# DanielaCourel/smoothed_particle_hydrodynamics

Measured on AMD Instinct MI355X. Metric: Mparticle-steps/sec (whole node), dam-break, higher is better.
Workload: dtype f32

## Files before the change

smoothed_particle_hydrodynamics_amd/csrc/cell_build.h:

```cpp
#pragma once

#include "sph_device.h"

#define SCAN_THREADS 256
#ifndef RANK_UNROLL
#define RANK_UNROLL 4
#endif
#ifndef RANK_BIG
#define RANK_BIG 512
#endif
#define RANK_CHUNK 4096
#define RANK_BIG_BLOCKS 64
#define SCAN_ITEMS 16
#define SCAN_TILE (SCAN_THREADS * SCAN_ITEMS)

__device__ __forceinline__ void count_cell_runs(uint32_t c, bool live, int i,
                                                uint32_t* __restrict__ cell_count,
                                                uint32_t* __restrict__ slot, uint32_t trash)
{
   live = live && c != trash;
   const int lane = threadIdx.x & (SPH_WAVE - 1);
   const uint32_t prev = __shfl_up(c, 1);
   const bool head = (lane == 0) || (prev != c);
   const unsigned long long heads = __ballot(head);
   const unsigned long long below = heads & ((lane == 63) ? ~0ull : ((1ull << (lane + 1)) - 1ull));
   const int head_lane = 63 - __clzll(below);
   const unsigned long long above = (head_lane == 63) ? 0ull : (heads >> (head_lane + 1));
   const int run_len = above ? (__ffsll((long long)above)) : (SPH_WAVE - head_lane);
   uint32_t base = 0;
   if (live && head) base = atomicAdd(&cell_count[c], (uint32_t)run_len);
   base = __shfl(base, head_lane);
   if (live) slot[i] = base + (uint32_t)(lane - head_lane);
}

template <bool WRITE_VOX, bool CHECK_DEAD>
__global__ void __launch_bounds__(256)
k_hash_count(const float4* __restrict__ posm, const float4* __restrict__ velp,
             int32_t* __restrict__ meta, CellGrid g, SlabZone zone, uint32_t* __restrict__ key,
             uint32_t* __restrict__ slot, uint32_t* __restrict__ cell_count,
             int32_t* __restrict__ vox)
{
   const int i = blockIdx.x * blockDim.x + threadIdx.x;
   const bool live = i < meta[META_N_IN];
   uint32_t c = 0xffffffffu;
   if (live) {
      const float4 p = posm[i];
      int cx, cy, cz;
      c = cell_of(g, p.x, p.y, p.z, cx, cy, cz);
      const bool carried = zone.drop_ghosts && i < meta[META_N_LIVE];
      const int ob = meta[META_OWN_BEGIN], oe = meta[META_OWN_END];
      const bool was_owned = i >= ob && i < oe;
      if (CHECK_DEAD && __float_as_uint(velp[i].w) == SPH_DEAD_ID) {
         c = (uint32_t)g.ncells;
      } else if (carried && !was_owned) {
         c = (uint32_t)g.ncells;
      } else if (c == (uint32_t)g.ncells) {
         if (!carried) atomicOr(&meta[META_ERRORS], 1);
      } else if (zone.early && carried) {
         const int lo_end = meta[META_BND_LO_END];
         const int hi_begin = max(meta[META_BND_HI_BEGIN], lo_end);
         if (i >= lo_end && i < hi_begin) {
            const int plane = cell_coord(p.z, g.inv, g.nz_global);
            if ((zone.have_left && plane < zone.lo + zone.halo) ||
                (zone.have_right && plane >= zone.hi - zone.halo))
               atomicOr(&meta[META_ERRORS], 8);
// ... 79 lines not shown
      for (int k = 0; k < SCAN_ITEMS / 4; k++) {
         const uint4 q = p[k];
         v[4 * k + 0] = q.x;
         v[4 * k + 1] = q.y;
         v[4 * k + 2] = q.z;
         v[4 * k + 3] = q.w;
      }
   } else {
#pragma unroll
      for (int k = 0; k < SCAN_ITEMS; k++) v[k] = (base + k < ncells) ? count[base + k] : 0u;
   }
#pragma unroll
   for (int k = 0; k < SCAN_ITEMS; k++) s += v[k];
   uint32_t before = 0;
   for (int t = threadIdx.x; t < (int)blockIdx.x; t += SCAN_THREADS) before += part[t];
   uint32_t carry;
   block_exclusive_scan(before, &carry);
   uint32_t total;
   uint32_t run = carry + block_exclusive_scan(s, &total);
   if (base + SCAN_ITEMS <= ncells) {
      uint4* o = reinterpret_cast<uint4*>(cell_start + base);
      uint4* z = reinterpret_cast<uint4*>(count + base);
#pragma unroll
      for (int k = 0; k < SCAN_ITEMS / 4; k++) {
         uint4 q;
         q.x = min(run, limit); run += v[4 * k + 0];
         q.y = min(run, limit); run += v[4 * k + 1];
         q.z = min(run, limit); run += v[4 * k + 2];
         q.w = min(run, limit); run += v[4 * k + 3];
         o[k] = q;
         if ((v[4 * k + 0] | v[4 * k + 1] | v[4 * k + 2] | v[4 * k + 3]) != 0u) z[k] = make_uint4(0, 0, 0, 0);
      }
   } else {
      for (int k = 0; k < SCAN_ITEMS; k++) {
         if (base + k < ncells) {
            cell_start[base + k] = min(run, limit);
            if (v[k] != 0u) count[base + k] = 0;
            run += v[k];
         }
      }
   }
   if (base <= ncells - 1 && ncells - 1 < base + SCAN_ITEMS) {
      cell_start[ncells] = min(run, limit);
      if (run > limit) atomicOr(&meta[META_ERRORS], 4);
   }
}

__global__ void __launch_bounds__(256)
k_scatter(const uint32_t* __restrict__ key, const uint32_t* __restrict__ slot,
          const uint32_t* __restrict__ cell_start, int32_t* __restrict__ meta,
          uint32_t* __restrict__ perm, int cells_per_plane, int ncells, int own_lo, int own_hi,
          int sum_lo, int sum_hi, int bnd_lo, int bnd_hi, int32_t* __restrict__ tile_stats,
          int32_t* __restrict__ clear_a, int32_t* __restrict__ clear_b,
          uint32_t* __restrict__ big_cells, uint32_t limit)
{
   const int i = blockIdx.x * blockDim.x + threadIdx.x;
   if (tile_stats && i < TSTAT_COUNT && i != TSTAT_BLOCKS) tile_stats[i] = 0;
   const int n_in = meta[META_N_IN];
   if (i < n_in) {
      const uint32_t c = key[i];
      if (c != (uint32_t)ncells) {
         const uint32_t first = cell_start[c], sl = slot[i];
         if (first + sl < limit) perm[first + sl] = (uint32_t)i;
         if (sl == 0u && cell_start[c + 1] - first > (uint32_t)RANK_BIG)
            big_cells[1u + atomicAdd(&big_cells[0], 1u)] = c;
      }
   }
   if (i == 0) {
      meta[META_N_LIVE] = (int)cell_start[ncells];
      meta[META_OWN_BEGIN] = (int)cell_start[own_lo * cells_per_plane];
      meta[META_OWN_END] = (int)cell_start[own_hi * cells_per_plane];
      meta[META_SUM_BEGIN] = (int)cell_start[sum_lo * cells_per_plane];
      meta[META_SUM_END] = (int)cell_start[sum_hi * cells_per_plane];
      meta[META_BND_LO_END] = (int)cell_start[bnd_lo * cells_per_plane];
      meta[META_BND_HI_BEGIN] = (int)cell_start[bnd_hi * cells_per_plane];
      if (clear_a) *clear_a = 0;
      if (clear_b) *clear_b = 0;
      if (tile_stats)
         tile_stats[TSTAT_BLOCKS] =
            (meta[META_SUM_END] - meta[META_SUM_BEGIN] + TILE_THREADS - 1) / TILE_THREADS;
   }
}

__global__ void __launch_bounds__(256)
k_rank_order(const uint32_t* __restrict__ perm, const uint32_t* __restrict__ key,
             const uint32_t* __restrict__ cell_start, const int32_t* __restrict__ meta,
             uint32_t* __restrict__ order)
{
   const int p = blockIdx.x * blockDim.x + threadIdx.x;
   if (p >= meta[META_N_IN]) return;
   const uint32_t i = perm[p];
   const uint32_t c = key[i];
   const uint32_t s = cell_start[c], e = cell_start[c + 1];
   if (e - s > (uint32_t)RANK_BIG) return;
   uint32_t rank = 0;
   for (uint32_t q0 = s; q0 < e; q0 += 8) {
      uint32_t other[8];
#pragma unroll
      for (int u = 0; u < 8; u++) other[u] = perm[q0 + u < e ? q0 + u : e - 1];
#pragma unroll
      for (int u = 0; u < 8; u++) rank += (q0 + u < e && other[u] < i) ? 1u : 0u;
   }
   order[s + rank] = i;
}

__device__ __forceinline__ void
rank_gather(int p, int block_p0, uint32_t* __restrict__ lds_id, const uint32_t* __restrict__ perm,
            const uint32_t* __restrict__ key, const uint32_t* __restrict__ cell_start,
            const int32_t* __restrict__ meta, int trash, const float4* __restrict__ posm_in,
            const float4* __restrict__ velp_in, float4* __restrict__ posm_out,
            float4* __restrict__ velp_out, uint32_t* __restrict__ remap = nullptr)
{
   const int n_in = (int)cell_start[trash];
   bool active = p < n_in;
   uint32_t i = 0, c = 0, s = 0, e = 0, id = 0;
   float4 v = make_float4(0.f, 0.f, 0.f, 0.f);
   if (active) {
      i = perm[p];
      c = key[i];
      v = velp_in[i];
      id = __float_as_uint(v.w);
   }
   lds_id[threadIdx.x] = id;
   if (active) {
      if (c == (uint32_t)trash) {
         active = false;
      } else {
         s = cell_start[c];
         e = cell_start[c + 1];
         if (e - s > (uint32_t)RANK_BIG) active = false;
      }
   }
   __syncthreads();
   if (!active) return;
   const uint32_t b0 = (uint32_t)block_p0;
   const uint32_t b1 = min(b0 + blockDim.x, (uint32_t)n_in);
   const uint32_t in_lo = max(s, b0), in_hi = min(e, b1);
   uint32_t rank = 0, same = 0;
   for (uint32_t q0 = in_lo; q0 < in_hi; q0 += 4) {
      uint32_t other[4];
#pragma unroll
      for (int u = 0; u < 4; u++) other[u] = lds_id[(q0 + u < in_hi ? q0 + u : in_hi - 1) - b0];
#pragma unroll
      for (int u = 0; u < 4; u++) {
         rank += (q0 + u < in_hi && other[u] < id) ? 1u : 0u;
         same += (q0 + u < in_hi && other[u] == id) ? 1u : 0u;
      }
   }
#pragma unroll
   for (int side = 0; side < 2; side++) {
      const uint32_t lo = side == 0 ? s : in_hi, hi = side == 0 ? in_lo : e;
      for (uint32_t q0 = lo; q0 < hi; q0 += RANK_UNROLL) {
         uint32_t other[RANK_UNROLL];
#pragma unroll
         for (int u = 0; u < RANK_UNROLL; u++) other[u] = perm[q0 + u < hi ? q0 + u : hi - 1];
#pragma unroll
         for (int u = 0; u < RANK_UNROLL; u++) other[u] = __float_as_uint(velp_in[other[u]].w);
#pragma unroll
         for (int u = 0; u < RANK_UNROLL; u++) {
            rank += (q0 + u < hi && other[u] < id) ? 1u : 0u;
            same += (q0 + u < hi && other[u] == id) ? 1u : 0u;
         }
      }
   }
   if (same > 1u) atomicOr(const_cast<int32_t*>(&meta[META_ERRORS]), 16);
   posm_out[s + rank] = posm_in[i];
   velp_out[s + rank] = v;
   if (remap) remap[i] = s + rank;
}

__global__ void __launch_bounds__(256)
k_rank_gather(const uint32_t* __restrict__ perm, const uint32_t* __restrict__ key,
              const uint32_t* __restrict__ cell_start, const int32_t* __restrict__ meta, int trash,
              const float4* __restrict__ posm_in, const float4* __restrict__ velp_in,
              float4* __restrict__ posm_out, float4* __restrict__ velp_out,
              uint32_t* __restrict__ remap)
{
   __shared__ uint32_t lds_id[256];
   rank_gather(blockIdx.x * blockDim.x + threadIdx.x, blockIdx.x * blockDim.x, lds_id, perm, key,
               cell_start, meta, trash, posm_in, velp_in, posm_out, velp_out, remap);
}

template <bool FULL>
__global__ void __launch_bounds__(256)
k_rank_big(const uint32_t* __restrict__ big_cells, const uint32_t* __restrict__ perm,
           const uint32_t* __restrict__ cell_start, const float4* __restrict__ posm_in,
           const float4* __restrict__ velp_in, float4* __restrict__ posm_out,
           float4* __restrict__ velp_out, uint32_t* __restrict__ order,
           uint32_t* __restrict__ scratch_key, uint32_t* __restrict__ scratch_src,
           uint32_t* __restrict__ remap)
{
   __shared__ uint32_t skey[RANK_CHUNK], ssrc[RANK_CHUNK];
   const int tid = threadIdx.x;
   const uint32_t nbig = big_cells[0];
   for (uint32_t b = blockIdx.x; b < nbig; b += gridDim.x) {
      const uint32_t c = big_cells[1u + b];
      const uint32_t s = cell_start[c], m = cell_start[c + 1] - s;
      const uint32_t nchunks = (m + RANK_CHUNK - 1) / RANK_CHUNK;
      for (uint32_t ch = 0; ch < nchunks; ch++) {
         const uint32_t base = ch * RANK_CHUNK;
         const uint32_t len = min((uint32_t)RANK_CHUNK, m - base);
         uint32_t padded = 256;
         while (padded < len) padded <<= 1;
         for (uint32_t t = tid; t < padded; t += 256) {
            uint32_t key = 0xffffffffu, src = 0u;
            if (t < len) {
               src = perm[s + base + t];
               key = FULL ? __float_as_uint(velp_in[src].w) : src;
            }
            skey[t] = key;
            ssrc[t] = src;
         }
         __syncthreads();
         for (uint32_t k2 = 2; k2 <= padded; k2 <<= 1) {
            for (uint32_t j = k2 >> 1; j > 0; j >>= 1) {
               for (uint32_t t = tid; t < padded; t += 256) {
                  const uint32_t partner = t ^ j;
                  if (partner > t) {
                     const bool up = (t & k2) == 0;
                     const uint32_t a = skey[t], bb = skey[partner];
                     if ((a > bb) == up) {
                        skey[t] = bb;
                        skey[partner] = a;
                        const uint32_t sa = ssrc[t];
                        ssrc[t] = ssrc[partner];
                        ssrc[partner] = sa;
                     }
                  }
               }
               __syncthreads();
            }
         }
         for (uint32_t t = tid; t < len; t += 256) {
            if (nchunks == 1) {
               const uint32_t src = ssrc[t];
               if (FULL) {
                  posm_out[s + t] = posm_in[src];
                  velp_out[s + t] = velp_in[src];
                  if (remap) remap[src] = s + t;
               } else {
                  order[s + t] = src;
               }
            } else {
               scratch_key[s + base + t] = skey[t];
               scratch_src[s + base + t] = ssrc[t];
            }
         }
         __syncthreads();
      }
      if (nchunks > 1) {
         for (uint32_t idx = tid; idx < m; idx += 256) {
            const uint32_t key = scratch_key[s + idx], mine = idx / RANK_CHUNK;
            uint32_t rank = idx % RANK_CHUNK;
            for (uint32_t ch = 0; ch < nchunks; ch++) {
               if (ch == mine) continue;
               const uint32_t* keys = scratch_key + s + ch * RANK_CHUNK;
               uint32_t lo = 0, hi = min((uint32_t)RANK_CHUNK, m - ch * RANK_CHUNK);
               while (lo < hi) {
                  const uint32_t mid = (lo + hi) >> 1;
                  if (keys[mid] < key) lo = mid + 1;
                  else hi = mid;
               }
               rank += lo;
            }
            const uint32_t src = scratch_src[s + idx];
            if (FULL) {
               posm_out[s + rank] = posm_in[src];
               velp_out[s + rank] = velp_in[src];
               if (remap) remap[src] = s + rank;
            } else {
               order[s + rank] = src;
            }
         }
         __syncthreads();
      }
   }
}

__global__ void __launch_bounds__(256)
k_permute_sums(const uint32_t* __restrict__ remap, const uint32_t* __restrict__ key,
               const int32_t* __restrict__ meta, uint32_t trash, const float* __restrict__ rho,
               const float4* __restrict__ acc, const int32_t* __restrict__ ncount,
               float* __restrict__ rho_out, float4* __restrict__ acc_out,
               int32_t* __restrict__ ncount_out)
{
   const int i = blockIdx.x * blockDim.x + threadIdx.x;
   if (i >= meta[META_N_IN] || key[i] == trash) return;
   const uint32_t j = remap[i];
   rho_out[j] = rho[i];
   acc_out[j] = acc[i];
   ncount_out[j] = ncount[i];
}
```

smoothed_particle_hydrodynamics_amd/csrc/context.h:

```cpp
#pragma once

#include <stdlib.h>
#include <string.h>

#include <memory>
#include <new>
#include <utility>

#include "cell_build.h"
#include "common_kernels.h"
#include "full_kernels.h"
#include "full_tiled.h"
#include "ref_kernels.h"
#include "sample_kernels.h"
#include "slab_kernels.h"
#include "slab_rccl.h"

namespace {

std::string g_create_error;

inline int div_up(int a, int b) { return (a + b - 1) / b; }

bool getenv_flag(const char* name)
// ... 65 lines not shown

struct SlabComm {
   ncclComm_t comm = nullptr;
   int rank = 0, nranks = 1;
   Stream stream;
   Event packed;
   Event arrived;
   DevBuf<void> send_left, send_right, recv_left, recv_right;
   int capacity_records = 0;
   int active_records = 0;
   size_t bytes = 0;
   DevBuf<int32_t> trim_word;
   bool primed = false;
   long long steps_run = 0;
   DevBuf<int32_t> fill_word;
   PinnedBuf<int32_t> fill_host;
   Event fill_arrived;
   bool fill_pending = false;
   int growths = 0;

   ~SlabComm()
   {
      const RcclApi* api = comm ? rccl_api(nullptr) : nullptr;
      if (api) (void)api->CommDestroy(comm);
   }
};
#define SLAB_GROW_EVERY 16

struct sph_hip_context {
   sph_hip_params prm;
   int mode = 0;
   int device = 0;
   int capacity = 0;
   int n = 0;
   int n_owned = 0;
   DevBuf<int32_t> meta;
   int plane_lo = 0, plane_hi = 0, halo = 0;
   hipStream_t stream = nullptr;
   Stream own_stream;
   Event ev[EV_RING][7];
   long long ev_steps = 0;
   std::string err;

   CellGrid grid;

   DevBuf<float4> posm[2];
   DevBuf<float4> velp[2];
   int cur = 0;

   DevBuf<uint32_t> key;
   DevBuf<uint32_t> slot;
   DevBuf<uint32_t> perm;
   DevBuf<uint32_t> order;
   DevBuf<uint32_t> cell_count;
   DevBuf<uint32_t> cell_start;
   DevBuf<uint32_t> scan_part;
   DevBuf<uint32_t> big_cells;
   int scan_tiles = 0;

   DevBuf<float> rho;
   DevBuf<float4> velB;
   DevBuf<float> auxc;
   DevBuf<float4> acc;
   DevBuf<int32_t> ncount;
   DevBuf<TileDesc> tile_desc;
   DevBuf<uint32_t> nlist;
   DevBuf<uint32_t> nlist_overflow;
   int fast = 0;
   int uniform_mass = 0;
   int use_tiled = 1;
   int prehashed = 0;
   int no_prehash = 0, no_fused_integrate = 0, no_fused_slab = 0;
   Stream chunk_stream;
   Event ev_chunk_fork, ev_chunk_join;
   int chunked_giveups = -1;
   int slab_fused = 0;
   void* slab_msgs[2] = {nullptr, nullptr};
   int slab_msg_capacity = 0;
   int had_exchange = 0;
   int may_hold_dead = 0;
   int early_exchange = 0;
   std::unique_ptr<SlabComm> comm;
   hipStream_t border_stream = nullptr;
   Event ev_density;
   Event ev_border;
   Event ev_pace[2];
   long long steps_enqueued = 0;
   int timing_level = 2;
   int timing_stride = 1;
   long long timing_seen = 0;
   int slab_step_level = 0;
   PinnedBuf<int> tile_feedback;
   DevBuf<int32_t> tile_stats;
   DevBuf<uint32_t> giveup_density;
   DevBuf<uint32_t> giveup_accel;
   int tile_cap_forced = 0;
   int tile_cap_accel = 0, tile_cap_density = 0;
   int list_cap = 0;
   int list_cap_max = 0;
   size_t list_blocks = 0;
   TileLevels density_levels = {}, accel_levels = {};
   TileCaps caps = {};
   int cand_kept[TILE_CANDS] = {0}, n_cand_kept = 0;

   DevBuf<int32_t> vox;
   DevBuf<uint32_t> nb;
// ... 123 lines not shown
   for (int b = 0; b < nbuf; b++) {
      CREATE_TRY(dev_alloc(ctx->posm[b], cap));
      CREATE_TRY(dev_alloc(ctx->velp[b], cap));
   }
   CREATE_TRY(dev_alloc(ctx->key, cap));
   CREATE_TRY(dev_alloc(ctx->slot, cap));
   CREATE_TRY(dev_alloc(ctx->perm, cap));
   const size_t cells_padded = (size_t)ctx->scan_tiles * SCAN_TILE + 16;
   CREATE_TRY(dev_alloc(ctx->cell_count, cells_padded));
   CREATE_TRY(dev_alloc(ctx->cell_start, cells_padded));
   CREATE_TRY(dev_alloc(ctx->scan_part, (size_t)ctx->scan_tiles + 1));
   CREATE_TRY(dev_alloc(ctx->big_cells, cap / RANK_BIG + 2));
   CREATE_TRY(hipMemsetAsync(ctx->big_cells, 0, sizeof(uint32_t), ctx->stream));
   CREATE_TRY(hipMemsetAsync(ctx->cell_count, 0, cells_padded * sizeof(uint32_t), ctx->stream));
   CREATE_TRY(hipMemsetAsync(ctx->cell_start, 0, cells_padded * sizeof(uint32_t), ctx->stream));
   CREATE_TRY(dev_alloc(ctx->rho, cap));
   CREATE_TRY(dev_alloc(ctx->acc, cap));
   CREATE_TRY(dev_alloc(ctx->ncount, cap));
   CREATE_TRY(hipMemsetAsync(ctx->rho, 0, cap * sizeof(float), ctx->stream));
   CREATE_TRY(hipMemsetAsync(ctx->acc, 0, cap * sizeof(float4), ctx->stream));
   CREATE_TRY(hipMemsetAsync(ctx->ncount, 0, cap * sizeof(int32_t), ctx->stream));
   CREATE_TRY(dev_alloc(ctx->meta, META_COUNT));
   CREATE_TRY(hipMemsetAsync(ctx->meta, 0, META_COUNT * sizeof(int32_t), ctx->stream));
   if (mode == SPH_HIP_MODE_FULL) {
      CREATE_TRY(dev_alloc(ctx->velB, cap));
      CREATE_TRY(dev_alloc(ctx->auxc, cap));
      CREATE_TRY(dev_alloc(ctx->tile_desc, (size_t)div_up(capacity, TILE_THREADS) + 1));
      ctx->list_cap = NLIST_CAP;
      ctx->list_cap_max = NLIST_CAP_MAX;
      if (const char* v = getenv("SPH_HIP_LIST_CAP")) {
         const int c = atoi(v) / 2 * 2;
         if (c > 0) ctx->list_cap = ctx->list_cap_max = c < 2 ? 2 : (c > NLIST_CAP_MAX ? NLIST_CAP_MAX : c);
      }
      ctx->list_blocks = (size_t)div_up(capacity, TILE_THREADS) + 1;
      const size_t nlist_words = ctx->list_blocks * list_rows(ctx->list_cap) * TILE_THREADS;
      CREATE_TRY(dev_alloc(ctx->nlist, nlist_words));
      CREATE_TRY(hipMemsetAsync(ctx->nlist, 0, nlist_words * sizeof(uint32_t), ctx->stream));
      CREATE_TRY(dev_alloc(ctx->nlist_overflow, (size_t)div_up(capacity, TILE_THREADS) + 1));
      if (const char* v = getenv("SPH_HIP_UNTILED")) ctx->use_tiled = (v[0] == '1') ? 0 : 1;
      CREATE_TRY(pinned_alloc(ctx->tile_feedback, TSTAT_COUNT));
      memset(ctx->tile_feedback, 0, TSTAT_COUNT * sizeof(int));
      CREATE_TRY(dev_alloc(ctx->tile_stats, TSTAT_COUNT));
      CREATE_TRY(hipMemsetAsync(ctx->tile_stats, 0, TSTAT_COUNT * sizeof(int32_t), ctx->stream));
      CREATE_TRY(dev_alloc(ctx->giveup_density, (size_t)div_up(capacity, TILE_THREADS) + 1));
      CREATE_TRY(dev_alloc(ctx->giveup_accel, (size_t)div_up(capacity, TILE_THREADS) + 1));
      CREATE_TRY(event_create(ctx->ev_density));
      CREATE_TRY(event_create(ctx->ev_border));
      if (const char* v = getenv("SPH_HIP_TILE_CAP")) {
         const int c = atoi(v);
         if (c > 0) ctx->tile_cap_forced = c < 256 ? 256 : (c > 8000 ? 8000 : c / 32 * 32);
      }
      if (const char* v = getenv("SPH_HIP_TILE_CAP_ACCEL")) ctx->tile_cap_accel = atoi(v) / 32 * 32;
      if (const char* v = getenv("SPH_HIP_TILE_CAP_DENSITY")) ctx->tile_cap_density = atoi(v) / 32 * 32;
   } else {
      CREATE_TRY(dev_alloc(ctx->order, cap));
      CREATE_TRY(dev_alloc(ctx->vox, cap * 3));
      CREATE_TRY(dev_alloc(ctx->nb, cap * (size_t)params->examine_count));
      CREATE_TRY(dev_alloc(ctx->nd, cap * (size_t)params->examine_count));
   }
   CREATE_TRY(dev_alloc(ctx->epart, (size_t)2 * ctx->eblocks + 2));
   CREATE_TRY(hipMemsetAsync(ctx->epart, 0, sizeof(double) * 2, ctx->stream));
   CREATE_TRY(dev_alloc(ctx->stats, 4));
   CREATE_TRY(pinned_alloc(ctx->err_watch, 4));
   for (int i = 0; i < 4; i++) ctx->err_watch[i] = 0;
   CREATE_TRY(event_create(ctx->watch_event));
   CREATE_TRY(dev_alloc(ctx->stage, cap * 12));
   CREATE_TRY(hipStreamSynchronize(ctx->stream));
#undef CREATE_TRY
   *out = ctx.release();
   return SPH_HIP_OK;
}

void destroy_impl(sph_hip_context* ctx)
{
   (void)hipSetDevice(ctx->device);
   if (ctx->stream) (void)hipStreamSynchronize(ctx->stream);
   if (ctx->comm && ctx->comm->stream) (void)hipStreamSynchronize(ctx->comm->stream);
   if (ctx->chunk_stream) (void)hipStreamSynchronize(ctx->chunk_stream);
   if (ctx->copy_stream) (void)hipStreamSynchronize(ctx->copy_stream);
   delete ctx;
}

}
```

smoothed_particle_hydrodynamics_amd/csrc/full_tiled.h:

```cpp
#pragma once

#include "launch_policy.h"
#include "common_kernels.h"
#include "full_kernels.h"
#include "slab_kernels.h"

#if defined(SPH_ABLATE) && !defined(SPH_DIAGNOSTIC_BUILD)
#error "SPH_ABLATE is for diagnostic builds only: add -DSPH_DIAGNOSTIC_BUILD (tools/build_variant.sh does)"
#endif

#ifdef SPH_TRIPCOUNT
#ifndef SPH_DIAGNOSTIC_BUILD
#error "SPH_TRIPCOUNT is for diagnostic builds only: add -DSPH_DIAGNOSTIC_BUILD"
#endif
enum {
   TRIP_D_WAVES = 0, TRIP_D_CHUNKS_W, TRIP_D_TEST8_W, TRIP_D_TEST8_L, TRIP_D_SLOTS_L, TRIP_D_POPS_W,
   TRIP_D_POPS_L, TRIP_D_POPLOOPS_W, TRIP_D_SUMTRIPS_W, TRIP_D_SUMSLOTS_W, TRIP_D_LISTED_L, TRIP_D_LANES_L,
   TRIP_A_WAVES = 16, TRIP_A_PTRIPS_W, TRIP_A_CNT_L, TRIP_A_VTRIPS_W, TRIP_A_NV_L, TRIP_A_LANES_L,
   TRIP_COUNT = 32
};
__device__ unsigned long long g_trip[TRIP_COUNT];
struct TripCounters {
   unsigned int v[16];
   __device__ TripCounters() { for (int i = 0; i < 16; i++) v[i] = 0; }
// ... 181 lines not shown
         len[k] = 0;
         if (hi >= lo) {
            G[k] = (int)cell_start[lo];
            len[k] = (int)cell_start[hi + 1] - G[k];
         }
      }
      int run = 0, chain_end = -1, chain_d = 0;
#pragma unroll
      for (int k = 0; k < 9; k++) {
         d.B[k] = run;
         if (len[k] == 0) {
            d.D[k] = run - G[k];
         } else if (G[k] <= chain_end) {
            const int seg_end = G[k] + len[k];
            d.D[k] = chain_d;
            if (seg_end > chain_end) {
               run += seg_end - chain_end;
               chain_end = seg_end;
            }
         } else {
            d.D[k] = chain_d = run - G[k];
            run += len[k];
            chain_end = G[k] + len[k];
         }
      }
      d.total = run;
      d.pad = 0;
      desc[tile] = d;
      most = run;
   }
   const bool lead = (threadIdx.x & (SPH_WAVE - 1)) == 0;
#pragma unroll
   for (int c = 0; c < TILE_CANDS; c++) {
      const int over = __popcll(__ballot(c < caps.n_cand && most > caps.cand[c]));
      if (lead && over) atomicAdd(&stats[TSTAT_OVER + c], over);
   }
   int wave_most = most;
#pragma unroll
   for (int o = SPH_WAVE / 2; o > 0; o >>= 1) wave_most = max(wave_most, __shfl_xor(wave_most, o));
   if (lead && wave_most > stats[TSTAT_MAX]) atomicMax(&stats[TSTAT_MAX], wave_most);
   if (most > caps.cap_density) giveup_density[atomicAdd(&stats[TSTAT_GIVEUP_DENSITY], 1)] = (uint32_t)tile;
   if (most > caps.cap_density || most > caps.cap_accel)
      giveup_accel[atomicAdd(&stats[TSTAT_GIVEUP_ACCEL], 1)] = (uint32_t)tile;
}

__global__ void __launch_bounds__(256)
k_rank_gather_tile_desc(int desc_blocks, int ntiles, const uint32_t* __restrict__ perm,
                        const uint32_t* __restrict__ key, const uint32_t* __restrict__ cell_start,
                        const int32_t* __restrict__ meta, CellGrid g,
                        const float4* __restrict__ posm_in, const float4* __restrict__ velp_in,
                        float4* __restrict__ posm_out, float4* __restrict__ velp_out,
                        TileDesc* __restrict__ desc, TileCaps caps, int32_t* __restrict__ stats,
                        uint32_t* __restrict__ giveup_density, uint32_t* __restrict__ giveup_accel,
                        uint32_t* __restrict__ remap)
{
   if ((int)blockIdx.x < desc_blocks) {
      tile_desc(blockIdx.x * blockDim.x + threadIdx.x, ntiles, perm, key, cell_start, meta, g, desc,
                caps, stats, giveup_density, giveup_accel);
      return;
   }
   __shared__ uint32_t lds_id[256];
   rank_gather((blockIdx.x - desc_blocks) * blockDim.x + threadIdx.x,
               (blockIdx.x - desc_blocks) * blockDim.x, lds_id, perm, key, cell_start, meta,
               g.ncells, posm_in, velp_in, posm_out, velp_out, remap);
}

__device__ __forceinline__ void tile_desc_load(const TileDesc* __restrict__ desc, int wg, TileDesc& sd)
{
   const int tid = threadIdx.x;
   if (tid < (int)(sizeof(TileDesc) / sizeof(int)))
      reinterpret_cast<int*>(&sd)[tid] = reinterpret_cast<const int*>(&desc[wg])[tid];
   __syncthreads();
}

__device__ __forceinline__ int xcd_workgroup(int block, int nblocks)
{
   const int q = nblocks / 8, r = nblocks % 8, x = block % 8;
   return (x < r ? x * (q + 1) : r * (q + 1) + (x - r) * q) + block / 8;
}

__device__ __forceinline__ void tile_load(const float4* __restrict__ posm, const TileDesc& sd,
                                          const TileLds& L)
{
   const int tid = threadIdx.x;
   const int total = sd.total;
   int B[9], D[9];
#pragma unroll
   for (int k = 0; k < 9; k++) {
      B[k] = sd.B[k];
      D[k] = sd.D[k];
   }
#if defined(SPH_ABLATE) && (SPH_ABLATE == 3 || SPH_ABLATE == 5)
   for (int base = 0; base < 0; base += TILE_BATCH * TILE_THREADS) {
#else
   for (int base = 0; base < total; base += TILE_BATCH * TILE_THREADS) {
#endif
      float4 buf[TILE_BATCH];
#pragma unroll
      for (int r = 0; r < TILE_BATCH; r++) {
         const int idx = min(base + tid + r * TILE_THREADS, total - 1);
         int d = D[0];
#pragma unroll
         for (int k = 1; k < 9; k++) d = (idx >= B[k]) ? D[k] : d;
         buf[r] = posm[idx - d];
      }
#pragma unroll
      for (int r = 0; r < TILE_BATCH; r++) {
         const int idx = base + tid + r * TILE_THREADS;
         if (idx < total) {
            L.x[idx] = buf[r].x;
            L.y[idx] = buf[r].y;
            L.z[idx] = buf[r].z;
         }
      }
   }
   __syncthreads();
}
// ... 1048 lines not shown
```

smoothed_particle_hydrodynamics_amd/csrc/launch.h:

```cpp
#pragma once

#include <math.h>

#include <type_traits>

#include "context.h"

namespace {

template <class F>
void bind_flags(F&& f) { f(); }
template <class F, class... Rest>
void bind_flags(F&& f, bool flag, Rest... rest)
{
   if (flag) bind_flags([&](auto... later) { f(std::true_type{}, later...); }, rest...);
   else bind_flags([&](auto... later) { f(std::false_type{}, later...); }, rest...);
}

PairConsts pair_consts(const sph_hip_params& p, bool fast)
{
   PairConsts k;
   k.h2 = p.h2;
   static const float screen = getenv("SPH_HIP_TEST_SCREEN") ? (float)atof(getenv("SPH_HIP_TEST_SCREEN"))
                                                             : TEST_SCREEN_FACTOR;
// ... 149 lines not shown

SlabZone slab_zone(const sph_hip_context* ctx)
{
   SlabZone z;
   z.lo = ctx->plane_lo;
   z.hi = ctx->plane_hi;
   z.halo = ctx->halo;
   z.have_left = ctx->plane_lo > 0;
   z.have_right = ctx->plane_hi < ctx->grid.nz_global;
   z.drop_ghosts = ctx->mode == SPH_HIP_MODE_FULL;
   z.early = ctx->early_exchange;
   return z;
}

int launch_cell_build(sph_hip_context* ctx, void* clear_left = nullptr, void* clear_right = nullptr,
                      bool keep_sums = false)
{
   const int n = ctx->n;
   if (n == 0) return SPH_HIP_OK;
   const int blocks = div_up(n, 256);
   const CellGrid g = ctx->grid;
   hipStream_t st = ctx->stream;
   const int cur = ctx->cur;
   const SlabZone zone = slab_zone(ctx);
   if (ctx->prehashed == 2) {
      ctx->prehashed = 0;
      hipLaunchKernelGGL(k_hash_tail, dim3(SLAB_PACK_BLOCKS), dim3(256), 0, st, ctx->posm[cur], ctx->meta, g,
                         ctx->key, ctx->slot, ctx->cell_count);
   } else if (ctx->prehashed) {
      ctx->prehashed = 0;
   } else {
      const bool ref = ctx->mode == SPH_HIP_MODE_REF;
      bind_flags([&](auto R, auto D) {
         if constexpr (!(R.value && D.value))
            hipLaunchKernelGGL((k_hash_count<R.value, D.value>), dim3(blocks), dim3(256), 0, st, ctx->posm[cur],
                               ctx->velp[cur], ctx->meta, g, zone, ctx->key, ctx->slot, ctx->cell_count,
                               R.value ? ctx->vox.get() : nullptr);
      }, ref, !ref && ctx->may_hold_dead != 0);
   }
   ctx->early_exchange = 0;
   ctx->may_hold_dead = 0;
   const int tiles = ctx->scan_tiles;
   const int ncells_scan = g.ncells + 1;
   hipLaunchKernelGGL(k_scan_reduce, dim3(tiles), dim3(SCAN_THREADS), 0, st, ctx->cell_count,
                      ncells_scan, ctx->scan_part);
   hipLaunchKernelGGL(k_scan_final, dim3(tiles), dim3(SCAN_THREADS), 0, st, ctx->cell_count,
                      ncells_scan, ctx->scan_part, ctx->cell_start, ctx->big_cells, (uint32_t)ctx->capacity,
                      ctx->meta);
   const PlaneRanges r = plane_ranges(ctx->plane_lo, ctx->plane_hi, g.z0, g.nz, ctx->halo, zone.have_left,
                                      zone.have_right);
   hipLaunchKernelGGL(k_scatter, dim3(blocks), dim3(256), 0, st, ctx->key, ctx->slot,
                      ctx->cell_start, ctx->meta, ctx->perm, g.nx * g.ny, g.ncells, r.own_lo, r.own_hi,
                      r.sum_lo, r.sum_hi, r.bnd_lo, r.bnd_hi, ctx->tile_stats, (int32_t*)clear_left,
                      (int32_t*)clear_right, ctx->big_cells, (uint32_t)ctx->capacity);
   uint32_t* scratch_key = reinterpret_cast<uint32_t*>(ctx->stage.get());
   uint32_t* scratch_src = scratch_key + ctx->capacity;
   uint32_t* remap = (keep_sums && ctx->mode == SPH_HIP_MODE_FULL && !ctx->had_exchange) ? ctx->slot : nullptr;
   if (ctx->mode == SPH_HIP_MODE_REF) {
      hipLaunchKernelGGL(k_rank_order, dim3(blocks), dim3(256), 0, st, ctx->perm, ctx->key,
                         ctx->cell_start, ctx->meta, ctx->order);
      hipLaunchKernelGGL(k_rank_big<false>, dim3(RANK_BIG_BLOCKS), dim3(256), 0, st, ctx->big_cells,
                         ctx->perm, ctx->cell_start, (const float4*)nullptr, (const float4*)nullptr,
                         (float4*)nullptr, (float4*)nullptr, ctx->order, scratch_key, scratch_src,
                         (uint32_t*)nullptr);
   } else {
      const int nxt = cur ^ 1;
      if (ctx->use_tiled) {
         static_assert(sizeof(TileDesc) == 20 * sizeof(int), "TileDesc is 20 ints");
         pick_tile_caps(ctx);
         const int ntiles = div_up(n, TILE_THREADS), desc_blocks = div_up(ntiles, 256);
         hipLaunchKernelGGL(k_rank_gather_tile_desc, dim3(desc_blocks + blocks), dim3(256), 0, st,
                            desc_blocks, ntiles, ctx->perm, ctx->key, ctx->cell_start, ctx->meta,
                            g, ctx->posm[cur], ctx->velp[cur], ctx->posm[nxt], ctx->velp[nxt],
                            ctx->tile_desc, ctx->caps, ctx->tile_stats, ctx->giveup_density,
                            ctx->giveup_accel, remap);
      } else {
         hipLaunchKernelGGL(k_rank_gather, dim3(blocks), dim3(256), 0, st, ctx->perm, ctx->key,
                            ctx->cell_start, ctx->meta, g.ncells, ctx->posm[cur], ctx->velp[cur],
                            ctx->posm[nxt], ctx->velp[nxt], remap);
      }
      hipLaunchKernelGGL(k_rank_big<true>, dim3(RANK_BIG_BLOCKS), dim3(256), 0, st, ctx->big_cells,
                         ctx->perm, ctx->cell_start, ctx->posm[cur], ctx->velp[cur], ctx->posm[nxt],
                         ctx->velp[nxt], (uint32_t*)nullptr, scratch_key, scratch_src, remap);
      if (remap) {
         float4* acc_t = reinterpret_cast<float4*>(ctx->stage.get() + ((2 * (size_t)ctx->capacity + 3) & ~(size_t)3));
         float* rho_t = reinterpret_cast<float*>(acc_t + (size_t)ctx->capacity);
         int32_t* cnt_t = reinterpret_cast<int32_t*>(rho_t + (size_t)ctx->capacity);
         hipLaunchKernelGGL(k_permute_sums, dim3(blocks), dim3(256), 0, st, remap, ctx->key, ctx->meta,
                            (uint32_t)g.ncells, ctx->rho, ctx->acc, ctx->ncount, rho_t, acc_t, cnt_t);
         SPH_TRY(hipMemcpyAsync(ctx->rho, rho_t, sizeof(float) * n, hipMemcpyDeviceToDevice, st));
         SPH_TRY(hipMemcpyAsync(ctx->acc, acc_t, sizeof(float4) * n, hipMemcpyDeviceToDevice, st));
         SPH_TRY(hipMemcpyAsync(ctx->ncount, cnt_t, sizeof(int32_t) * n, hipMemcpyDeviceToDevice, st));
      }
      ctx->cur = nxt;
   }
   SPH_TRY(hipGetLastError());
   return SPH_HIP_OK;
}

int launch_find_neighbors(sph_hip_context* ctx)
{
   if (ctx->mode != SPH_HIP_MODE_REF || ctx->n == 0) return SPH_HIP_OK;
   const sph_hip_params& p = ctx->prm;
   hipLaunchKernelGGL(k_ref_find_neighbors, dim3(div_up(ctx->n, 256)), dim3(256), 0, ctx->stream,
                      ctx->posm[0], ctx->vox, ctx->cell_start, ctx->order, ctx->n, p.cells_x,
                      p.cells_y, p.cells_z, p.h, p.htimes2, p.h2, p.sim_scale, p.examine_count,
                      ctx->nb, ctx->nd, ctx->ncount);
   SPH_TRY(hipGetLastError());
   return SPH_HIP_OK;
}

struct SlabFused {
   void* left;
   void* right;
   int capacity;
};

void launch_density_tiled(sph_hip_context* ctx, bool unit, int blocks, const PairConsts& k)
{
   const int cap = ctx->caps.cap_density;
   const size_t lds = (size_t)(cap + TILE_PAD) * DENSITY_TILE_BYTES;
   const bool whole = ctx->plane_lo == 0 && ctx->plane_hi == ctx->grid.nz_global;
   double* epart_clear = whole ? nullptr : ctx->epart + 2;
   const int reported = ((volatile int*)ctx->tile_feedback)[TSTAT_GIVEUP_DENSITY];
   const bool chunked = ctx->chunked_giveups == 1 || (ctx->chunked_giveups < 0 && reported >= 32);
   hipStream_t side = ctx->stream;
   if (chunked) {
      if (!ctx->chunk_stream) {
         if (hipStreamCreateWithFlags(ctx->chunk_stream.out(), hipStreamNonBlocking) != hipSuccess ||
             event_create(ctx->ev_chunk_fork) != hipSuccess || event_create(ctx->ev_chunk_join) != hipSuccess) {
            (void)hipGetLastError();
            ctx->chunk_stream.reset();
         }
      }
      if (ctx->chunk_stream && hipEventRecord(ctx->ev_chunk_fork, ctx->stream) == hipSuccess &&
          hipStreamWaitEvent(ctx->chunk_stream, ctx->ev_chunk_fork, 0) == hipSuccess)
// ... 244 lines not shown
```

smoothed_particle_hydrodynamics_amd/csrc/launch_policy.h:

```cpp
#pragma once

#include <stdint.h>

#include "../../include/sph_hip.h"

#ifndef TILE_THREADS
#define TILE_THREADS 256
#endif
#define TILE_PAD 32
#define TILE_CAP_MAX (4096 - TILE_PAD)
#define TILE_CAP_MAX_WIDE (16384 - TILE_PAD)

#define TILE_CANDS 12
enum {
   TSTAT_OVER = 0,
   TSTAT_BLOCKS = 12,
   TSTAT_MAX = 13,
   TSTAT_GIVEUP_DENSITY = 14,
   TSTAT_GIVEUP_ACCEL = 15,
   TSTAT_NO_LIST = 16,
   TSTAT_COUNT = 17
};
struct TileCaps {
   int cand[TILE_CANDS];
// ... 109 lines not shown
   if (forced > 0) {
      caps.cap_density = caps.cap_accel = forced;
      if (forced_accel >= 256 && forced_accel < caps.cap_accel) caps.cap_accel = forced_accel;
      if (forced_density >= 256 && forced_density < caps.cap_density) caps.cap_density = forced_density;
      caps.wide = forced > TILE_CAP_MAX;
      return;
   }
   caps.cap_density = pick_level(caps, fb, density, DENSITY_THR, DENSITY_GIVEUP_COST);
   caps.cap_accel = pick_level(caps, fb, accel, ACCEL_THR, ACCEL_UNTILED_COST,
                               over_at(caps, fb, caps.cap_density), ACCEL_LISTED_COST);
   caps.wide = caps.cap_density > TILE_CAP_MAX || caps.cap_accel > TILE_CAP_MAX;
}

inline bool lists_should_grow(int without, int blocks)
{
   return without > 64 && without > blocks * (TILE_THREADS / 256);
}

inline int smaller_list_cap(int want) { return (want / 2 - 1) & ~1; }

inline int grown_active_records(long long most, int active, int capacity)
{
   const bool grow = most * SLAB_GROW_FILL_DEN > (long long)active * SLAB_GROW_FILL_NUM && active < capacity;
   return grow ? capacity : active;
}

inline int trim_records(int most, float slack, int extra, int capacity)
{
   const double want_d = (double)most * (double)slack + (double)extra;
   const int want = want_d > (double)capacity ? capacity : (int)want_d;
   return want < 1 ? 1 : want;
}

struct PlaneRanges {
   int own_lo, own_hi;
   int sum_lo, sum_hi;
   int bnd_lo, bnd_hi;
};

inline PlaneRanges plane_ranges(int plane_lo, int plane_hi, int z0, int nz, int halo, bool have_left,
                                bool have_right)
{
   PlaneRanges r;
   r.own_lo = plane_lo - z0;
   r.own_hi = plane_hi - z0;
   r.sum_lo = r.own_lo - 1 < 0 ? 0 : r.own_lo - 1;
   r.sum_hi = r.own_hi + 1 > nz ? nz : r.own_hi + 1;
   const int border = halo + 1;
   r.bnd_lo = !have_left ? r.own_lo : (r.own_lo + border < r.own_hi ? r.own_lo + border : r.own_hi);
   r.bnd_hi = !have_right ? r.own_hi : (r.own_hi - border > r.own_lo ? r.own_hi - border : r.own_lo);
   return r;
}

inline int phase_event(bool full_mode, int k)
{
   if (k == 4) return 3;
   if (k == 2 && full_mode) return 1;
   return k;
}

inline bool records_boundary(int level, bool full_mode, int k)
{
   if (level == SPH_HIP_TIMING_PHASES) return phase_event(full_mode, k) == k;
   return level == SPH_HIP_TIMING_SUMS && (k == 1 || k == 5);
}

inline int next_step_level(bool timed, int level, long long& seen, int stride)
{
   if (!timed || level == SPH_HIP_TIMING_OFF) return SPH_HIP_TIMING_OFF;
   const bool sample = (seen++ % stride) == 0;
   return sample ? level : SPH_HIP_TIMING_OFF;
}
```

Baseline: 4760.

## Fuse big-cell ranking into rank-gather launches and precompute sorted cell keys

The separate k_rank_big launch is folded into k_rank_order, k_rank_gather and k_rank_gather_tile_desc: the first 64 blocks handle big cells and the remaining blocks do small-cell ranking. This removes one kernel launch and its serialization point per step. k_scatter also writes a sorted_key array so the gather reads the cell key coalesced instead of doing a dependent key[i] lookup, and posm is loaded early. To fit both paths into one kernel, RANK_CHUNK is halved to 2048, which raises LDS use for the small-rank blocks and may make big-cell sorting slower.

```diff
diff --git a/smoothed_particle_hydrodynamics_amd/csrc/cell_build.h b/smoothed_particle_hydrodynamics_amd/csrc/cell_build.h
--- a/smoothed_particle_hydrodynamics_amd/csrc/cell_build.h
+++ b/smoothed_particle_hydrodynamics_amd/csrc/cell_build.h
@@ -9,8 +9,7 @@
 #ifndef RANK_BIG
 #define RANK_BIG 512
 #endif
-#define RANK_CHUNK 4096
-#define RANK_BIG_BLOCKS 64
+#define RANK_CHUNK 2048
 #define SCAN_ITEMS 16
 #define SCAN_TILE (SCAN_THREADS * SCAN_ITEMS)
 
@@ -196,7 +195,7 @@
           uint32_t* __restrict__ perm, int cells_per_plane, int ncells, int own_lo, int own_hi,
           int sum_lo, int sum_hi, int bnd_lo, int bnd_hi, int32_t* __restrict__ tile_stats,
           int32_t* __restrict__ clear_a, int32_t* __restrict__ clear_b,
-          uint32_t* __restrict__ big_cells, uint32_t limit)
+          uint32_t* __restrict__ big_cells, uint32_t limit, uint32_t* __restrict__ sorted_key)
 {
    const int i = blockIdx.x * blockDim.x + threadIdx.x;
    if (tile_stats && i < TSTAT_COUNT && i != TSTAT_BLOCKS) tile_stats[i] = 0;
@@ -204,9 +203,12 @@
    if (i < n_in) {
       const uint32_t c = key[i];
       if (c != (uint32_t)ncells) {
-         const uint32_t first = cell_start[c], sl = slot[i];
-         if (first + sl < limit) perm[first + sl] = (uint32_t)i;
-         if (sl == 0u && cell_start[c + 1] - first > (uint32_t)RANK_BIG)
+         const uint32_t first = cell_start[c], last = cell_start[c + 1], sl = slot[i];
+         if (first + sl < limit) {
+            perm[first + sl] = (uint32_t)i;
+            if (sorted_key) sorted_key[first + sl] = c;
+         }
+         if (sl == 0u && last - first > (uint32_t)RANK_BIG)
             big_cells[1u + atomicAdd(&big_cells[0], 1u)] = c;
       }
    }
@@ -226,118 +228,20 @@
    }
 }
 
-__global__ void __launch_bounds__(256)
-k_rank_order(const uint32_t* __restrict__ perm, const uint32_t* __restrict__ key,
-             const uint32_t* __restrict__ cell_start, const int32_t* __restrict__ meta,
-             uint32_t* __restrict__ order)
-{
-   const int p = blockIdx.x * blockDim.x + threadIdx.x;
-   if (p >= meta[META_N_IN]) return;
-   const uint32_t i = perm[p];
-   const uint32_t c = key[i];
-   const uint32_t s = cell_start[c], e = cell_start[c + 1];
-   if (e - s > (uint32_t)RANK_BIG) return;
-   uint32_t rank = 0;
-   for (uint32_t q0 = s; q0 < e; q0 += 8) {
-      uint32_t other[8];
-#pragma unroll
-      for (int u = 0; u < 8; u++) other[u] = perm[q0 + u < e ? q0 + u : e - 1];
-#pragma unroll
-      for (int u = 0; u < 8; u++) rank += (q0 + u < e && other[u] < i) ? 1u : 0u;
-   }
-   order[s + rank] = i;
-}
-
+template <bool FULL>
 __device__ __forceinline__ void
-rank_gather(int p, int block_p0, uint32_t* __restrict__ lds_id, const uint32_t* __restrict__ perm,
-            const uint32_t* __restrict__ key, const uint32_t* __restrict__ cell_start,
-            const int32_t* __restrict__ meta, int trash, const float4* __restrict__ posm_in,
-            const float4* __restrict__ velp_in, float4* __restrict__ posm_out,
-            float4* __restrict__ velp_out, uint32_t* __restrict__ remap = nullptr)
-{
-   const int n_in = (int)cell_start[trash];
-   bool active = p < n_in;
-   uint32_t i = 0, c = 0, s = 0, e = 0, id = 0;
-   float4 v = make_float4(0.f, 0.f, 0.f, 0.f);
-   if (active) {
-      i = perm[p];
-      c = key[i];
-      v = velp_in[i];
-      id = __float_as_uint(v.w);
-   }
-   lds_id[threadIdx.x] = id;
-   if (active) {
-      if (c == (uint32_t)trash) {
-         active = false;
-      } else {
-         s = cell_start[c];
-         e = cell_start[c + 1];
-         if (e - s > (uint32_t)RANK_BIG) active = false;
-      }
-   }
-   __syncthreads();
-   if (!active) return;
-   const uint32_t b0 = (uint32_t)block_p0;
-   const uint32_t b1 = min(b0 + blockDim.x, (uint32_t)n_in);
-   const uint32_t in_lo = max(s, b0), in_hi = min(e, b1);
-   uint32_t rank = 0, same = 0;
-   for (uint32_t q0 = in_lo; q0 < in_hi; q0 += 4) {
-      uint32_t other[4];
-#pragma unroll
-      for (int u = 0; u < 4; u++) other[u] = lds_id[(q0 + u < in_hi ? q0 + u : in_hi - 1) - b0];
-#pragma unroll
-      for (int u = 0; u < 4; u++) {
-         rank += (q0 + u < in_hi && other[u] < id) ? 1u : 0u;
-         same += (q0 + u < in_hi && other[u] == id) ? 1u : 0u;
-      }
-   }
-#pragma unroll
-   for (int side = 0; side < 2; side++) {
-      const uint32_t lo = side == 0 ? s : in_hi, hi = side == 0 ? in_lo : e;
-      for (uint32_t q0 = lo; q0 < hi; q0 += RANK_UNROLL) {
-         uint32_t other[RANK_UNROLL];
-#pragma unroll
-         for (int u = 0; u < RANK_UNROLL; u++) other[u] = perm[q0 + u < hi ? q0 + u : hi - 1];
-#pragma unroll
-         for (int u = 0; u < RANK_UNROLL; u++) other[u] = __float_as_uint(velp_in[other[u]].w);
-#pragma unroll
-         for (int u = 0; u < RANK_UNROLL; u++) {
-            rank += (q0 + u < hi && other[u] < id) ? 1u : 0u;
-            same += (q0 + u < hi && other[u] == id) ? 1u : 0u;
-         }
-      }
-   }
-   if (same > 1u) atomicOr(const_cast<int32_t*>(&meta[META_ERRORS]), 16);
-   posm_out[s + rank] = posm_in[i];
-   velp_out[s + rank] = v;
-   if (remap) remap[i] = s + rank;
-}
-
-__global__ void __launch_bounds__(256)
-k_rank_gather(const uint32_t* __restrict__ perm, const uint32_t* __restrict__ key,
-              const uint32_t* __restrict__ cell_start, const int32_t* __restrict__ meta, int trash,
-              const float4* __restrict__ posm_in, const float4* __restrict__ velp_in,
-              float4* __restrict__ posm_out, float4* __restrict__ velp_out,
-              uint32_t* __restrict__ remap)
-{
-   __shared__ uint32_t lds_id[256];
-   rank_gather(blockIdx.x * blockDim.x + threadIdx.x, blockIdx.x * blockDim.x, lds_id, perm, key,
-               cell_start, meta, trash, posm_in, velp_in, posm_out, velp_out, remap);
-}
-
-template <bool FULL>
-__global__ void __launch_bounds__(256)
-k_rank_big(const uint32_t* __restrict__ big_cells, const uint32_t* __restrict__ perm,
-           const uint32_t* __restrict__ cell_start, const float4* __restrict__ posm_in,
-           const float4* __restrict__ velp_in, float4* __restrict__ posm_out,
-           float4* __restrict__ velp_out, uint32_t* __restrict__ order,
-           uint32_t* __restrict__ scratch_key, uint32_t* __restrict__ scratch_src,
-           uint32_t* __restrict__ remap)
-{
-   __shared__ uint32_t skey[RANK_CHUNK], ssrc[RANK_CHUNK];
+rank_big(uint32_t wg, uint32_t* __restrict__ lds, const uint32_t* __restrict__ big_cells,
+         const uint32_t* __restrict__ perm, const uint32_t* __restrict__ cell_start,
+         const float4* __restrict__ posm_in, const float4* __restrict__ velp_in,
+         float4* __restrict__ posm_out, float4* __restrict__ velp_out, uint32_t* __restrict__ order,
+         uint32_t* __restrict__ scratch_key, uint32_t* __restrict__ scratch_src,
+         uint32_t* __restrict__ remap)
+{
+   uint32_t* __restrict__ skey = lds;
+   uint32_t* __restrict__ ssrc = lds + RANK_CHUNK;
    const int tid = threadIdx.x;
    const uint32_t nbig = big_cells[0];
-   for (uint32_t b = blockIdx.x; b < nbig; b += gridDim.x) {
+   for (uint32_t b = wg; b < nbig; b += RANK_BIG_BLOCKS) {
       const uint32_t c = big_cells[1u + b];
       const uint32_t s = cell_start[c], m = cell_start[c + 1] - s;
       const uint32_t nchunks = (m + RANK_CHUNK - 1) / RANK_CHUNK;
@@ -421,6 +325,115 @@
    }
 }
 
+
+__global__ void __launch_bounds__(256)
+k_rank_order(const uint32_t* __restrict__ perm, const uint32_t* __restrict__ key,
+             const uint32_t* __restrict__ cell_start, const int32_t* __restrict__ meta,
+             uint32_t* __restrict__ order, const uint32_t* __restrict__ big_cells,
+             uint32_t* __restrict__ scratch_key, uint32_t* __restrict__ scratch_src)
+{
+   __shared__ uint32_t lds[2 * RANK_CHUNK];
+   if (blockIdx.x < RANK_BIG_BLOCKS) {
+      rank_big<false>(blockIdx.x, lds, big_cells, perm, cell_start, nullptr, nullptr, nullptr, nullptr,
+                      order, scratch_key, scratch_src, nullptr);
+      return;
+   }
+   const int p = (blockIdx.x - RANK_BIG_BLOCKS) * blockDim.x + threadIdx.x;
+   if (p >= meta[META_N_IN]) return;
+   const uint32_t i = perm[p];
+   const uint32_t c = key[i];
+   const uint32_t s = cell_start[c], e = cell_start[c + 1];
+   if (e - s > (uint32_t)RANK_BIG) return;
+   uint32_t rank = 0;
+   for (uint32_t q0 = s; q0 < e; q0 += 8) {
+      uint32_t other[8];
+#pragma unroll
+      for (int u = 0; u < 8; u++) other[u] = perm[q0 + u < e ? q0 + u : e - 1];
+#pragma unroll
+      for (int u = 0; u < 8; u++) rank += (q0 + u < e && other[u] < i) ? 1u : 0u;
+   }
+   order[s + rank] = i;
+}
+
+__device__ __forceinline__ void
+rank_gather(int p, int block_p0, uint32_t* __restrict__ lds_id, const uint32_t* __restrict__ perm,
+            const uint32_t* __restrict__ sorted_key, const uint32_t* __restrict__ cell_start,
+            const int32_t* __restrict__ meta, int trash, const float4* __restrict__ posm_in,
+            const float4* __restrict__ velp_in, float4* __restrict__ posm_out,
+            float4* __restrict__ velp_out, uint32_t* __restrict__ remap = nullptr)
+{
+   const int n_in = (int)cell_start[trash];
+   bool active = p < n_in;
+   uint32_t i = 0, s = 0, e = 0, id = 0;
+   float4 v = make_float4(0.f, 0.f, 0.f, 0.f), x = v;
+   if (active) {
+      i = perm[p];
+      const uint32_t c = sorted_key[p];
+      s = cell_start[c];
+      e = cell_start[c + 1];
+      v = velp_in[i];
+      x = posm_in[i];
+      id = __float_as_uint(v.w);
+   }
+   lds_id[threadIdx.x] = id;
+   if (active && e - s > (uint32_t)RANK_BIG) active = false;
+   __syncthreads();
+   if (!active) return;
+   const uint32_t b0 = (uint32_t)block_p0;
+   const uint32_t b1 = min(b0 + blockDim.x, (uint32_t)n_in);
+   const uint32_t in_lo = max(s, b0), in_hi = min(e, b1);
+   uint32_t rank = 0, same = 0;
+   for (uint32_t q0 = in_lo; q0 < in_hi; q0 += 4) {
+      uint32_t other[4];
+#pragma unroll
+      for (int u = 0; u < 4; u++) other[u] = lds_id[(q0 + u < in_hi ? q0 + u : in_hi - 1) - b0];
+#pragma unroll
+      for (int u = 0; u < 4; u++) {
+         rank += (q0 + u < in_hi && other[u] < id) ? 1u : 0u;
+         same += (q0 + u < in_hi && other[u] == id) ? 1u : 0u;
+      }
+   }
+#pragma unroll
+   for (int side = 0; side < 2; side++) {
+      const uint32_t lo = side == 0 ? s : in_hi, hi = side == 0 ? in_lo : e;
+      for (uint32_t q0 = lo; q0 < hi; q0 += RANK_UNROLL) {
+         uint32_t other[RANK_UNROLL];
+#pragma unroll
+         for (int u = 0; u < RANK_UNROLL; u++) other[u] = perm[q0 + u < hi ? q0 + u : hi - 1];
+#pragma unroll
+         for (int u = 0; u < RANK_UNROLL; u++) other[u] = __float_as_uint(velp_in[other[u]].w);
+#pragma unroll
+         for (int u = 0; u < RANK_UNROLL; u++) {
+            rank += (q0 + u < hi && other[u] < id) ? 1u : 0u;
+            same += (q0 + u < hi && other[u] == id) ? 1u : 0u;
+         }
+      }
+   }
+   if (same > 1u) atomicOr(const_cast<int32_t*>(&meta[META_ERRORS]), 16);
+   posm_out[s + rank] = x;
+   velp_out[s + rank] = v;
+   if (remap) remap[i] = s + rank;
+}
+
+__global__ void __launch_bounds__(256)
+k_rank_gather(const uint32_t* __restrict__ perm, const uint32_t* __restrict__ sorted_key,
+              const uint32_t* __restrict__ cell_start, const int32_t* __restrict__ meta, int trash,
+              const float4* __restrict__ posm_in, const float4* __restrict__ velp_in,
+              float4* __restrict__ posm_out, float4* __restrict__ velp_out,
+              uint32_t* __restrict__ remap, const uint32_t* __restrict__ big_cells,
+              uint32_t* __restrict__ scratch_key, uint32_t* __restrict__ scratch_src)
+{
+   __shared__ uint32_t lds[2 * RANK_CHUNK];
+   if (blockIdx.x < RANK_BIG_BLOCKS) {
+      rank_big<true>(blockIdx.x, lds, big_cells, perm, cell_start, posm_in, velp_in, posm_out, velp_out,
+                     nullptr, scratch_key, scratch_src, remap);
+      return;
+   }
+   const int b = blockIdx.x - RANK_BIG_BLOCKS;
+   rank_gather(b * blockDim.x + threadIdx.x, b * blockDim.x, lds, perm, sorted_key, cell_start, meta, trash,
+               posm_in, velp_in, posm_out, velp_out, remap);
+}
+
 __global__ void __launch_bounds__(256)
 k_permute_sums(const uint32_t* __restrict__ remap, const uint32_t* __restrict__ key,
                const int32_t* __restrict__ meta, uint32_t trash, const float* __restrict__ rho,
diff --git a/smoothed_particle_hydrodynamics_amd/csrc/context.h b/smoothed_particle_hydrodynamics_amd/csrc/context.h
--- a/smoothed_particle_hydrodynamics_amd/csrc/context.h
+++ b/smoothed_particle_hydrodynamics_amd/csrc/context.h
@@ -141,6 +141,7 @@
    DevBuf<uint32_t> slot;
    DevBuf<uint32_t> perm;
    DevBuf<uint32_t> order;
+   DevBuf<uint32_t> sorted_key;
    DevBuf<uint32_t> cell_count;
    DevBuf<uint32_t> cell_start;
    DevBuf<uint32_t> scan_part;
@@ -370,6 +371,8 @@
       }
       if (const char* v = getenv("SPH_HIP_TILE_CAP_ACCEL")) ctx->tile_cap_accel = atoi(v) / 32 * 32;
       if (const char* v = getenv("SPH_HIP_TILE_CAP_DENSITY")) ctx->tile_cap_density = atoi(v) / 32 * 32;
+      CREATE_TRY(dev_alloc(ctx->sorted_key, cap));
+      CREATE_TRY(hipMemsetAsync(ctx->sorted_key, 0, cap * sizeof(uint32_t), ctx->stream));
    } else {
       CREATE_TRY(dev_alloc(ctx->order, cap));
       CREATE_TRY(dev_alloc(ctx->vox, cap * 3));
diff --git a/smoothed_particle_hydrodynamics_amd/csrc/full_tiled.h b/smoothed_particle_hydrodynamics_amd/csrc/full_tiled.h
--- a/smoothed_particle_hydrodynamics_amd/csrc/full_tiled.h
+++ b/smoothed_particle_hydrodynamics_amd/csrc/full_tiled.h
@@ -257,17 +257,24 @@
                         float4* __restrict__ posm_out, float4* __restrict__ velp_out,
                         TileDesc* __restrict__ desc, TileCaps caps, int32_t* __restrict__ stats,
                         uint32_t* __restrict__ giveup_density, uint32_t* __restrict__ giveup_accel,
-                        uint32_t* __restrict__ remap)
-{
-   if ((int)blockIdx.x < desc_blocks) {
-      tile_desc(blockIdx.x * blockDim.x + threadIdx.x, ntiles, perm, key, cell_start, meta, g, desc,
-                caps, stats, giveup_density, giveup_accel);
+                        uint32_t* __restrict__ remap, const uint32_t* __restrict__ big_cells,
+                        uint32_t* __restrict__ scratch_key, uint32_t* __restrict__ scratch_src,
+                        const uint32_t* __restrict__ sorted_key)
+{
+   __shared__ uint32_t lds[2 * RANK_CHUNK];
+   if (blockIdx.x < RANK_BIG_BLOCKS) {
+      rank_big<true>(blockIdx.x, lds, big_cells, perm, cell_start, posm_in, velp_in, posm_out, velp_out,
+                     nullptr, scratch_key, scratch_src, remap);
       return;
    }
-   __shared__ uint32_t lds_id[256];
-   rank_gather((blockIdx.x - desc_blocks) * blockDim.x + threadIdx.x,
-               (blockIdx.x - desc_blocks) * blockDim.x, lds_id, perm, key, cell_start, meta,
-               g.ncells, posm_in, velp_in, posm_out, velp_out, remap);
+   const int b = (int)blockIdx.x - RANK_BIG_BLOCKS;
+   if (b < desc_blocks) {
+      tile_desc(b * blockDim.x + threadIdx.x, ntiles, perm, key, cell_start, meta, g, desc, caps, stats,
+                giveup_density, giveup_accel);
+      return;
+   }
+   rank_gather((b - desc_blocks) * blockDim.x + threadIdx.x, (b - desc_blocks) * blockDim.x, lds, perm,
+               sorted_key, cell_start, meta, g.ncells, posm_in, velp_in, posm_out, velp_out, remap);
 }
 
 __device__ __forceinline__ void tile_desc_load(const TileDesc* __restrict__ desc, int wg, TileDesc& sd)
diff --git a/smoothed_particle_hydrodynamics_amd/csrc/launch.h b/smoothed_particle_hydrodynamics_amd/csrc/launch.h
--- a/smoothed_particle_hydrodynamics_amd/csrc/launch.h
+++ b/smoothed_particle_hydrodynamics_amd/csrc/launch.h
@@ -225,36 +225,31 @@
    hipLaunchKernelGGL(k_scatter, dim3(blocks), dim3(256), 0, st, ctx->key, ctx->slot,
                       ctx->cell_start, ctx->meta, ctx->perm, g.nx * g.ny, g.ncells, r.own_lo, r.own_hi,
                       r.sum_lo, r.sum_hi, r.bnd_lo, r.bnd_hi, ctx->tile_stats, (int32_t*)clear_left,
-                      (int32_t*)clear_right, ctx->big_cells, (uint32_t)ctx->capacity);
+                      (int32_t*)clear_right, ctx->big_cells, (uint32_t)ctx->capacity,
+                      ctx->mode == SPH_HIP_MODE_REF ? nullptr : ctx->sorted_key.get());
    uint32_t* scratch_key = reinterpret_cast<uint32_t*>(ctx->stage.get());
    uint32_t* scratch_src = scratch_key + ctx->capacity;
    uint32_t* remap = (keep_sums && ctx->mode == SPH_HIP_MODE_FULL && !ctx->had_exchange) ? ctx->slot : nullptr;
    if (ctx->mode == SPH_HIP_MODE_REF) {
-      hipLaunchKernelGGL(k_rank_order, dim3(blocks), dim3(256), 0, st, ctx->perm, ctx->key,
-                         ctx->cell_start, ctx->meta, ctx->order);
-      hipLaunchKernelGGL(k_rank_big<false>, dim3(RANK_BIG_BLOCKS), dim3(256), 0, st, ctx->big_cells,
-                         ctx->perm, ctx->cell_start, (const float4*)nullptr, (const float4*)nullptr,
-                         (float4*)nullptr, (float4*)nullptr, ctx->order, scratch_key, scratch_src,
-                         (uint32_t*)nullptr);
+      hipLaunchKernelGGL(k_rank_order, dim3(rank_grid(n, 0).total), dim3(256), 0, st, ctx->perm, ctx->key,
+                         ctx->cell_start, ctx->meta, ctx->order, ctx->big_cells, scratch_key, scratch_src);
    } else {
       const int nxt = cur ^ 1;
       if (ctx->use_tiled) {
          static_assert(sizeof(TileDesc) == 20 * sizeof(int), "TileDesc is 20 ints");
          pick_tile_caps(ctx);
          const int ntiles = div_up(n, TILE_THREADS), desc_blocks = div_up(ntiles, 256);
-         hipLaunchKernelGGL(k_rank_gather_tile_desc, dim3(desc_blocks + blocks), dim3(256), 0, st,
+         hipLaunchKernelGGL(k_rank_gather_tile_desc, dim3(rank_grid(n, desc_blocks).total), dim3(256), 0, st,
                             desc_blocks, ntiles, ctx->perm, ctx->key, ctx->cell_start, ctx->meta,
                             g, ctx->posm[cur], ctx->velp[cur], ctx->posm[nxt], ctx->velp[nxt],
                             ctx->tile_desc, ctx->caps, ctx->tile_stats, ctx->giveup_density,
-                            ctx->giveup_accel, remap);
+                            ctx->giveup_accel, remap, ctx->big_cells, scratch_key, scratch_src,
+                            ctx->sorted_key.get());
       } else {
-         hipLaunchKernelGGL(k_rank_gather, dim3(blocks), dim3(256), 0, st, ctx->perm, ctx->key,
+         hipLaunchKernelGGL(k_rank_gather, dim3(rank_grid(n, 0).total), dim3(256), 0, st, ctx->perm, ctx->sorted_key.get(),
                             ctx->cell_start, ctx->meta, g.ncells, ctx->posm[cur], ctx->velp[cur],
-                            ctx->posm[nxt], ctx->velp[nxt], remap);
-      }
-      hipLaunchKernelGGL(k_rank_big<true>, dim3(RANK_BIG_BLOCKS), dim3(256), 0, st, ctx->big_cells,
-                         ctx->perm, ctx->cell_start, ctx->posm[cur], ctx->velp[cur], ctx->posm[nxt],
-                         ctx->velp[nxt], (uint32_t*)nullptr, scratch_key, scratch_src, remap);
+                            ctx->posm[nxt], ctx->velp[nxt], remap, ctx->big_cells, scratch_key, scratch_src);
+      }
       if (remap) {
          float4* acc_t = reinterpret_cast<float4*>(ctx->stage.get() + ((2 * (size_t)ctx->capacity + 3) & ~(size_t)3));
          float* rho_t = reinterpret_cast<float*>(acc_t + (size_t)ctx->capacity);
diff --git a/smoothed_particle_hydrodynamics_amd/csrc/launch_policy.h b/smoothed_particle_hydrodynamics_amd/csrc/launch_policy.h
--- a/smoothed_particle_hydrodynamics_amd/csrc/launch_policy.h
+++ b/smoothed_particle_hydrodynamics_amd/csrc/launch_policy.h
@@ -185,6 +185,20 @@
    return r;
 }
 
+#define RANK_BIG_BLOCKS 64
+struct RankGrid {
+   int big, desc, rank, total;
+};
+inline RankGrid rank_grid(int n, int desc_blocks)
+{
+   RankGrid r;
+   r.big = RANK_BIG_BLOCKS;
+   r.desc = desc_blocks;
+   r.rank = (n + 255) / 256;
+   r.total = r.big + r.desc + r.rank;
+   return r;
+}
+
 inline int phase_event(bool full_mode, int k)
 {
    if (k == 4) return 3;
```

Result: no change. 4773, median of 6 (+0.3%).
